# kubagalecki/L3STER

Measured on AMD Instinct MI355X. Metric: DOF/s for MF operator apply (Diffusion3D, hex p=6), higher is better.
Workload: dtype f64

## Files before the change

l3ster_amd/csrc/device/sumfact_fast.hpp:

```cpp
#ifndef L3K_DEVICE_SUMFACT_FAST_HPP
#define L3K_DEVICE_SUMFACT_FAST_HPP

#include "sumfact_apply.hpp"

#include <cstdio>
#include <cstdlib>
#include <type_traits>

namespace l3k::dev
{
template < int NIN, int NOUT, bool ANTI, bool ACC >
__device__ __forceinline__ void sweepEO(const double (&in)[NIN], double (&out)[NOUT], const double* __restrict__ eo)
{
    constexpr int HI = NIN / 2, HO = NOUT / 2, RI = (NIN + 1) / 2, RO = (NOUT + 1) / 2;
    const double* We = eo;
    const double* Wo = eo + RI * RO;
    double        e[RI], o[HI > 0 ? HI : 1];
#pragma unroll
    for (int r = 0; r < HI; ++r)
    {
        e[r] = in[r] + in[NIN - 1 - r];
        o[r] = in[r] - in[NIN - 1 - r];
    }
    if constexpr (NIN % 2)
        e[HI] = in[HI];
#pragma unroll
    for (int q = 0; q < HO; ++q)
    {
        double A = 0.;
#pragma unroll
        for (int r = 0; r < RI; ++r)
            A += e[r] * We[r * RO + q];
        if constexpr (ACC)
        {
            double lo = A;
#pragma unroll
            for (int r = 0; r < HI; ++r)
                lo += o[r] * Wo[r * RO + q];
            out[q] += lo;
            out[NOUT - 1 - q] += ANTI ? lo - 2. * A : 2. * A - lo;
        }
        else
        {
            double lo = A;
#pragma unroll
            for (int r = 0; r < HI; ++r)
                lo += o[r] * Wo[r * RO + q];
            out[q]            = lo;
            out[NOUT - 1 - q] = ANTI ? lo - 2. * A : 2. * A - lo;
        }
    }
    if constexpr (NOUT % 2)
    {
        double m = 0.;
        if constexpr (ANTI)
        {
#pragma unroll
            for (int r = 0; r < HI; ++r)
                m += o[r] * Wo[r * RO + HO];
        }
        else
        {
#pragma unroll
            for (int r = 0; r < RI; ++r)
                m += e[r] * We[r * RO + HO];
        }
        out[HO] = ACC ? out[HO] + m : m;
    }
}

template < int NIN, int NOUT, bool ANTI, bool ACC >
__device__ __forceinline__ void sweepEOSecond(bool live, const double (&in)[NIN], double (&out)[NOUT], const double* __restrict__ eo)
{
    if (live)
        sweepEO< NIN, NOUT, ANTI, ACC >(in, out, eo);
    else if constexpr (!ACC)
    {
#pragma unroll
        for (int q = 0; q < NOUT; ++q)
            out[q] = 0.;
    }
}

template < int N1, int NQ >
struct FastTables
{
    static constexpr int HN = (N1 + 1) / 2, HQ = (NQ + 1) / 2;
    double               eoI[2 * HN * HQ], eoC[2 * HQ * HQ], eoIt[2 * HQ * HN], eoCt[2 * HQ * HQ], qw[NQ], qx[NQ];
};

__device__ __forceinline__ int opaqueZero()
{
    int z;
    asm volatile("s_mov_b32 %0, 0" : "=s"(z) : : "memory");
    return z;
}
__device__ __forceinline__ int opaqueCopy(int x)
{
    int y;
    asm volatile("v_mov_b32 %0, %1" : "=v"(y) : "v"(x));
    return y;
}
__device__ __forceinline__ double opaqueCopy(double x)
{
    double y;
    asm volatile("v_mov_b64 %0, %1" : "=v"(y) : "v"(x));
    return y;
}
template < int N >
__device__ __forceinline__ void loadTable(double (&t)[N], const double* src)
{
#pragma unroll
    for (int i = 0; i < N; ++i)
        t[i] = src[i];
    __builtin_amdgcn_sched_barrier(0);
}
__device__ __forceinline__ void stageFence()
{
    __builtin_amdgcn_fence(__ATOMIC_RELEASE, "wavefront");
    __builtin_amdgcn_wave_barrier();
    __builtin_amdgcn_fence(__ATOMIC_ACQUIRE, "wavefront");
}

#ifdef L3K_ABLATION
#define L3K_STAMP(k)                                                                                                   \
    do                                                                                                                 \
    {                                                                                                                  \
        if (a.stamps != nullptr && blockIdx.x == 0 && stamp_it < 256)                                                  \
        {                                                                                                              \
            const long long t_ = __builtin_readcyclecounter();                                                         \
            if (lane == 0)                                                                                             \
                a.stamps[stamp_it * 16 + (k)] = t_;                                                                    \
        }                                                                                                              \
    } while (0)
#else
#define L3K_STAMP(k)                                                                                                   \
    do                                                                                                                 \
    {                                                                                                                  \
    } while (0)
#endif

#ifndef L3K_FAST_MIN_WAVES
#define L3K_FAST_MIN_WAVES 2
#endif
template < typename K >
constexpr bool kernelUsesFieldDers()
{
    if constexpr (requires { K::field_derivatives; })
        return K::field_derivatives;
    else
        return true;
}

template < int U >
__device__ __forceinline__ uint32_t dirichletBits(const uint8_t* __restrict__ mask, int64_t node)
{
    if constexpr (U == 4)
    {
        const uint32_t w = *reinterpret_cast< const uint32_t* >(mask + node * 4);
        return ((w & 0xffu) ? 1u : 0u) | ((w & 0xff00u) ? 2u : 0u) | ((w & 0xff0000u) ? 4u : 0u) | ((w & 0xff000000u) ? 8u : 0u);
    }
    else if constexpr (U == 2)
    {
        const uint32_t w = *reinterpret_cast< const uint16_t* >(mask + node * 2);
        return ((w & 0xffu) ? 1u : 0u) | ((w & 0xff00u) ? 2u : 0u);
    }
    else
    {
        uint32_t dm = 0;
#pragma unroll
        for (int u = 0; u < U; ++u)
            dm |= uint32_t(mask[node * U + u] != 0) << u;
        return dm;
    }
}

template < typename K, int NQ_, int NFD >
constexpr int kernelWavesPerSimd()
{
    if constexpr (requires { K::waves_per_simd; })
        return K::waves_per_simd;
    else
        return K::params.n_unknowns == 1 && NQ_ * NFD <= 36 ? 3 : L3K_FAST_MIN_WAVES;
}

template < typename K, int P, int NQ >
struct FastCfg
{
    static constexpr int N1 = P + 1, M = cmax(N1, NQ), TEAM = M * M, NN = N1 * N1 * N1;
    static constexpr int U = K::params.n_unknowns, F = K::params.n_fields, NF = U + F;
    static constexpr int NG = (NF + 1) / 2;
    static constexpr int UG = (U + 1) / 2;
    static constexpr int EW = 64 / TEAM > 0 ? 64 / TEAM : 1;
#ifdef L3K_FAST_PS
    static constexpr int PS = M == 7 ? L3K_FAST_PS : M * M, OS = PS * M;
#else
    static constexpr int PS_PAD = M == 8 ? 65 : (M == 6 ? 41 : (M == 4 ? 19 : M * M));
    static constexpr int ldsWith(int ps)
    {
        const int ng = (NF + 1) / 2, dg = kernelUsesFieldDers< K >() ? ng : (U + 1) / 2, os = ps * M;
        const bool alias = dg < ng && ng - dg >= dg;
        return 8 * EW * ((alias ? 2 * ng * os : 2 * ng * os + 2 * dg * os) + 26) + 16 * N1 * N1;
    }
    static constexpr int PS = ldsWith(PS_PAD) <= 64 * 1024 ? PS_PAD : M * M, OS = PS * M;
#endif
    static constexpr int    DG       = kernelUsesFieldDers< K >() ? NG : UG;
    static constexpr int    DF       = kernelUsesFieldDers< K >() ? NF : U;
    static constexpr int    BUF_D    = 2 * NG * OS;
    static constexpr int    BUFB_D   = 2 * DG * OS;
    static constexpr bool   ALIAS_B  = DG < NG && NG - DG >= DG;
    static constexpr int    OFF_B    = ALIAS_B ? 2 * DG * OS : BUF_D;
    static constexpr int    OFF_V    = ALIAS_B ? BUF_D : BUF_D + BUFB_D;
    static constexpr int    TEAM_D   = OFF_V + 24 + 2;
    static constexpr int    SLOT_B   = 16 * N1 * N1;
    static constexpr size_t lds      = sizeof(double) * size_t(EW) * TEAM_D + SLOT_B;
#ifndef L3K_FAST_PS
    static_assert(lds == size_t(ldsWith(PS)));
#endif
    static constexpr int    SG       = (64 / EW) / U * U;
    static constexpr int    NSH      = NN - (N1 - 2) * (N1 - 2) * (N1 - 2);
    static constexpr bool   feasible = TEAM <= 64 && lds <= 64 * 1024 && NF * cmax(N1, NQ) <= 64 && NN * U <= BUFB_D && N1 <= 8 && SG >= U;
    static constexpr int waves_by_lds = int((160 * 1024) / (lds > 0 ? lds : 1));
    static constexpr int min_waves    = waves_by_lds <= 4 ? 1 : (waves_by_lds <= 8 ? cmin(2, kernelWavesPerSimd< K, NQ, NF + DF >()) : kernelWavesPerSimd< K, NQ, NF + DF >());
    static constexpr int wavesPerSimd(bool multi) { return multi ? cmin(2, min_waves) : min_waves; }
    static constexpr int read_block   = NG;
    static constexpr bool multi_column = EW > 1;
};

template < typename K, int P, int NQ, bool SPLIT, bool ENERGY, bool AFFINE = false, bool MULTI = false, bool STRIDED = false, bool RHS = false >
__global__ __launch_bounds__(64, (FastCfg< K, P, NQ >::wavesPerSimd(MULTI))) void sumfactFastKernel(const ElemArgs a, const K kern, int64_t n_batches,
                                                        int xcd_chunk, const FastTables< P + 1, NQ > tab)
{
    using Cfg = FastCfg< K, P, NQ >;
    constexpr int N1 = Cfg::N1, M = Cfg::M, PS = Cfg::PS, OS = Cfg::OS, TEAM = Cfg::TEAM, EW = Cfg::EW;
    constexpr int U = Cfg::U, F = Cfg::F, NF = Cfg::NF, NG = Cfg::NG, UG = Cfg::UG, NN = N1 * N1 * N1;
    constexpr int DG = Cfg::DG, DF = Cfg::DF;
    static_assert(!STRIDED || (!ENERGY && !AFFINE && !MULTI));
    static_assert(!RHS || (!ENERGY && !AFFINE && !MULTI && !STRIDED));
    [[maybe_unused]] const int dpn = a.dofs_per_node;
    auto dirBits = [&](int64_t node) -> uint32_t {
        if constexpr (STRIDED)
        {
            uint32_t dm = 0;
#pragma unroll
            for (int u = 0; u < U; ++u)
                dm |= uint32_t(a.dirichlet[node * dpn + a.field_inds[u]] != 0) << u;
            return dm;
        }
        else
            return dirichletBits< U >(a.dirichlet, node);
    };
#if defined(L3K_FLAGGED_SCATTER)
    constexpr bool ENERGY_AT_END = false;
#elif defined(L3K_ENERGY_AT_END)
    constexpr bool ENERGY_AT_END = L3K_ENERGY_AT_END != 0;
#else
    constexpr bool ENERGY_AT_END = EW == 1;
#endif
    constexpr int HN = (N1 + 1) / 2, HQ = (NQ + 1) / 2;
    constexpr int GB = Cfg::read_block;
    constexpr bool INPLACE = DG < NG;
    auto          at = [](int c, int b, int a_) { return b * PS + a_ * M + c; };

    extern __shared__ double lds[];
    const int                lane = threadIdx.x;
    const int                team = lane / TEAM, l = lane - team * TEAM;
    const bool               worker = team < EW && l < cmax(N1 * N1, cmax(N1 * NQ, NQ * NQ));
    constexpr int            SG     = Cfg::SG;
    double* const            base = lds + size_t(worker ? team : 0) * Cfg::TEAM_D;
    double2* const           bufA = reinterpret_cast< double2* >(base);
    double2* const           bufB = reinterpret_cast< double2* >(base + Cfg::OFF_B);
    double* const            vs   = base + Cfg::OFF_V;

    const double* const eoI  = tab.eoI;
    const double* const eoC  = tab.eoC;
    const double* const eoIt = tab.eoIt;
    const double* const eoCt = tab.eoCt;
    const double* const qw   = tab.qw;
    const double* const qp   = tab.qx;

    const int  i1 = l % N1, j1 = l / N1;
    const bool on_nn = worker && (N1 == NQ ? true : l < N1 * N1);
    const int  iq = l % N1, kq = l / N1;
    const int  qa = l % NQ, qb = l / NQ;

    auto ldg = [&](const double2* buf, int g, int idx) { return buf[g * OS + idx]; };
    auto stg = [&](double2* buf, int g, int idx, double x0, double x1) { buf[g * OS + idx] = make_double2(x0, x1); };

    const int nb     = static_cast< int >(n_batches);
    const int by_xcd = xcd_chunk > 0;
    const int stride = by_xcd ? int(gridDim.x) >> 3 : int(gridDim.x);
    const int first  = by_xcd ? int(blockIdx.x & 7) * xcd_chunk : 0;
    const int last   = by_xcd ? (first + xcd_chunk < nb ? first + xcd_chunk : nb) : nb;
    const bool dyn     = a.work_counters != nullptr;
    const bool sharded = by_xcd || (gridDim.x & 7u) == 0;
    int        victim  = sharded ? int(blockIdx.x & 7u) : 0, switches = 0;
    auto       vBase   = [&](int v) { return by_xcd ? v * xcd_chunk : v; };
    auto       vLimit  = [&](int v) { return by_xcd ? (v * xcd_chunk + xcd_chunk < nb ? v * xcd_chunk + xcd_chunk : nb) : nb; };
    const int  dyn_step = by_xcd || !sharded ? 1 : 8;
    auto       drawTicket = [&]() -> uint32_t {
        uint32_t t = 0;
        if (dyn && lane == 0)
            t = __hip_atomic_fetch_add(a.work_counters + 32 * victim, 1u, __ATOMIC_RELAXED, __HIP_MEMORY_SCOPE_AGENT);
        return t;
    };
    auto ticketBatch = [&](uint32_t t) {
        int b = vBase(victim) + int(__builtin_amdgcn_readfirstlane(t)) * dyn_step;
        while (b >= vLimit(victim))
        {
            if (!by_xcd || ++switches > 7)
                return nb;
            victim = (victim + 1) & 7;
            b      = vBase(victim) + int(__builtin_amdgcn_readfirstlane(drawTicket())) * dyn_step;
        }
        return b;
    };
    const int lim   = dyn ? nb : last;
    int       batch = dyn ? ticketBatch(drawTicket()) : first + (by_xcd ? int(blockIdx.x >> 3) : int(blockIdx.x));
    uint32_t      ids_cur[N1], ids_nxt[N1];
    double        xn[N1][U];
    double        fn[N1][F > 0 ? F : 1];
    uint32_t      dm_nxt[N1];
    const int64_t n_owned_nodes = a.n_owned_dofs / (STRIDED ? a.dofs_per_node : U);
    auto          elemOf = [&](int b) { return a.elem_begin + int64_t(b) * EW + team; };
    auto          valid  = [&](int b) { return (b < lim) & on_nn & ((int64_t(b) * EW + team) < a.elem_count); };
    const bool have_flags = a.elem_flags != nullptr;
    auto       loadIds    = [&](int batch, uint32_t (&ids)[N1], uint32_t& flag) {
        const int lane_o = opaqueCopy(lane), steam = lane_o / SG;
        uint32_t  fg = 0, fs = 0;
        if (have_flags && batch < lim)
        {
            if (steam < EW && (int64_t(batch) * EW + steam) < a.elem_count)
                fs = a.elem_flags[a.elem_begin + int64_t(batch) * EW + steam];
            if constexpr (EW == 1)
                fg = fs;
            else if (worker && (int64_t(batch) * EW + team) < a.elem_count)
                fg = a.elem_flags[elemOf(batch)];
        }
        flag = ((fg & 1u) ? 1u : 0u) | ((fs & 1u) ? 2u : 0u);
        if (valid(batch))
        {
            const uint32_t* en = a.elem_nodes + elemOf(batch) * NN + (lane_o - team * TEAM);
#pragma unroll
            for (int k = 0; k < N1; ++k)
                ids[k] = en[k * N1 * N1];
        }
    };
    [[maybe_unused]] int col = 0;
    auto loadX = [&](bool mine, const uint32_t (&ids)[N1], bool flagged) {
        if (!mine)
            return;
        const double* const ax  = MULTI ? a.x + size_t(col) * a.ldx : a.x;
        const double* const axg = MULTI && SPLIT ? a.xg + size_t(col) * a.ldxg : a.xg;
#pragma unroll
        for (int k = 0; k < N1; ++k)
        {
            const int64_t node = ids[k];
            const double* p    = STRIDED ? (!SPLIT || node < n_owned_nodes ? ax + node * dpn : axg + (node - n_owned_nodes) * dpn)
                                         : (!SPLIT || node < n_owned_nodes ? ax + node * U : axg + (node - n_owned_nodes) * U);
            if constexpr (RHS)
            {
                const uint32_t dm = flagged ? dirBits(node) : 0u;
#pragma unroll
                for (int u = 0; u < U; ++u)
                    xn[k][u] = (dm >> u) & 1u ? a.dirichlet_vals[node * U + u] : 0.;
            }
            else if constexpr (STRIDED)
            {
#pragma unroll
                for (int u = 0; u < U; ++u)
                    xn[k][u] = p[a.field_inds[u]];
            }
            else if constexpr (U % 2 == 0)
            {
#pragma unroll
                for (int hh = 0; hh < U / 2; ++hh)
                {
                    const double2 t = (L3K_DBG(a) & 2) ? make_double2(1e-9 * double(node), 1e-9)
                                                  : *reinterpret_cast< const double2* >(p + 2 * hh);
                    xn[k][2 * hh]     = t.x;
                    xn[k][2 * hh + 1] = t.y;
                }
            }
            else
            {
#pragma unroll
                for (int u = 0; u < U; ++u)
                    xn[k][u] = (L3K_DBG(a) & 2) ? 1e-9 * double(node) : p[u];
            }
            dm_nxt[k] = !RHS && flagged ? dirBits(node) : 0u;
#pragma unroll
            for (int f = 0; f < F; ++f)
                fn[k][f] = a.fields[node + f * a.ldf];
        }
    };

    const double eta_l = qp[qa < NQ ? qa : 0], zeta_l = qp[qb < NQ ? qb : 0];
    const double wyz_l = qw[qa < NQ ? qa : 0] * qw[qb < NQ ? qb : 0];

    uint4* const slotRows = reinterpret_cast< uint4* >(lds + size_t(EW) * Cfg::TEAM_D);
    if (lane < N1 * N1)
        slotRows[lane] = reinterpret_cast< const uint4* >(a.slot_tab)[lane];
    if constexpr (ENERGY)
        if (worker && l == 0)
            vs[24] = 0.;
    stageFence();
    uint32_t flag_cur, flag_nxt = 0;
    loadIds(batch, ids_cur, flag_cur);

    [[maybe_unused]] int stamp_it = 0;
#ifdef L3K_ABLATION
    if (a.stamps != nullptr && blockIdx.x < 4096 && lane == 0)
        a.stamps[256 * 16 + 2 * blockIdx.x] = __builtin_readcyclecounter();
#endif
    while (batch < lim)
    {
        const uint32_t ticket = drawTicket();
        L3K_STAMP(0);
        const bool act = (int64_t(batch) * EW + team) < a.elem_count;
        const bool w_all = worker & act;
        const bool w_nn = N1 == NQ ? w_all : (w_all & (l < N1 * N1)), w_nq = N1 == NQ ? w_all : (w_all & (l < N1 * NQ)),
                   w_qq = N1 == NQ ? w_all : (w_all & (l < NQ * NQ));
        int        batch_next = 0;
        col                   = 0;
        do
        {
        if (w_all)
        {
        loadX(w_nn, ids_cur, RHS ? (a.dirichlet_vals != nullptr && ((flag_cur & 1u) != 0 || !have_flags)) : (flag_cur & 1u) != 0);
        double u0[N1][2 * NG];
        if (w_nn)
        {
#pragma unroll
            for (int k = 0; k < N1; ++k)
            {
#pragma unroll
                for (int u = 0; u < U; ++u)
                    u0[k][u] = xn[k][u];
                if (!RHS && (flag_cur & 1u) != 0)
                {
#pragma unroll
                    for (int u = 0; u < U; ++u)
                        u0[k][u] = (dm_nxt[k] >> u) & 1u ? 0. : u0[k][u];
                }
#pragma unroll
                for (int f = 0; f < F; ++f)
                    u0[k][U + f] = fn[k][f];
                if constexpr (NF % 2)
                    u0[k][NF] = 0.;
            }
        }
        constexpr bool VREG = TEAM >= 24;
        double         vreg = 0.;
        if constexpr (VREG)
        {
            if (l < 24)
                vreg = a.elem_verts[elemOf(batch) * 24 + opaqueCopy(l)];
        }
        else
        {
            for (int t = opaqueCopy(l); t < 24; t += TEAM)
                vs[t] = a.elem_verts[elemOf(batch) * 24 + t];
        }

        if (w_nn)
        {
            double tI[2 * HN * HQ];
            loadTable(tI, eoI + opaqueZero());
#pragma unroll
            for (int g = 0; g < NG; ++g)
            {
                double in0[N1], in1[N1], o0[NQ], o1[NQ];
#pragma unroll
                for (int k = 0; k < N1; ++k)
                {
                    in0[k] = u0[k][2 * g];
                    in1[k] = u0[k][2 * g + 1];
                }
                sweepEO< N1, NQ, false, false >(in0, o0, tI);
                sweepEOSecond< N1, NQ, false, false >(2 * g + 1 < NF, in1, o1, tI);
#pragma unroll
                for (int q = 0; q < NQ; ++q)
                    stg(bufA, g, at(i1, j1, q), o0[q], o1[q]);
            }
        }
        stageFence();
        L3K_STAMP(1);
        if (w_nq)
        {
            double tI[2 * HN * HQ];
            loadTable(tI, eoI + opaqueZero());
#pragma unroll
            for (int gb = 0; gb < NG; gb += GB)
            {
            double in0[GB][N1], in1[GB][N1];
#pragma unroll
            for (int g = gb; g < gb + GB && g < NG; ++g)
#pragma unroll
                for (int j = 0; j < N1; ++j)
                {
                    const double2 t = ldg(bufA, g, at(iq, j, kq));
                    in0[g - gb][j] = t.x;
                    in1[g - gb][j] = t.y;
                }
#pragma unroll
            for (int g = gb; g < gb + GB && g < NG; ++g)
            {
                double o0[NQ], o1[NQ];
                sweepEO< N1, NQ, false, false >(in0[g - gb], o0, tI);
                sweepEOSecond< N1, NQ, false, false >(2 * g + 1 < NF, in1[g - gb], o1, tI);
#pragma unroll
                for (int q = 0; q < NQ; ++q)
                    stg(INPLACE ? bufA : bufB, g, at(iq, q, kq), o0[q], o1[q]);
            }
            }
        }
        stageFence();
        L3K_STAMP(2);
        double v[NQ][2 * NG], dxi[NQ][2 * NG];
        if (w_qq)
        {
            double tI[2 * HN * HQ];
            loadTable(tI, eoI + opaqueZero());
#pragma unroll
            for (int gb = 0; gb < NG; gb += GB)
            {
            double in0[GB][N1], in1[GB][N1];
#pragma unroll
            for (int g = gb; g < gb + GB && g < NG; ++g)
#pragma unroll
                for (int i = 0; i < N1; ++i)
                {
                    const double2 t = ldg(INPLACE ? bufA : bufB, g, at(i, qa, qb));
                    in0[g - gb][i] = t.x;
                    in1[g - gb][i] = t.y;
                }
#pragma unroll
            for (int g = gb; g < gb + GB && g < NG; ++g)
            {
                double o0[NQ], o1[NQ];
                sweepEO< N1, NQ, false, false >(in0[g - gb], o0, tI);
                sweepEOSecond< N1, NQ, false, false >(2 * g + 1 < NF, in1[g - gb], o1, tI);
#pragma unroll
                for (int q = 0; q < NQ; ++q)
                {
                    v[q][2 * g]     = o0[q];
                    v[q][2 * g + 1] = o1[q];
                    if (g < DG)
                        stg(bufA, g, at(q, qa, qb), o0[q], o1[q]);
                }
            }
            }
            double tC[2 * HQ * HQ];
            loadTable(tC, eoC + opaqueZero());
#pragma unroll
            for (int o = 0; o < DF; ++o)
            {
                double in[NQ], der[NQ];
#pragma unroll
                for (int q = 0; q < NQ; ++q)
                    in[q] = v[q][o];
                sweepEO< NQ, NQ, true, false >(in, der, tC);
#pragma unroll
                for (int q = 0; q < NQ; ++q)
                    dxi[q][o] = der[q];
            }
        }
        stageFence();
        L3K_STAMP(3);
        if (w_qq)
        {
            double tC[2 * HQ * HQ];
            loadTable(tC, eoC + opaqueZero());
#pragma unroll
            for (int gb = 0; gb < DG; gb += GB)
            {
            double in0[GB][NQ], in1[GB][NQ];
#pragma unroll
            for (int g = gb; g < gb + GB && g < DG; ++g)
#pragma unroll
                for (int q = 0; q < NQ; ++q)
                {
                    const double2 t = ldg(bufA, g, at(qa, q, qb));
                    in0[g - gb][q] = t.x;
                    in1[g - gb][q] = t.y;
                }
#pragma unroll
            for (int g = gb; g < gb + GB && g < DG; ++g)
            {
                double o0[NQ], o1[NQ];
                sweepEO< NQ, NQ, true, false >(in0[g - gb], o0, tC);
                sweepEOSecond< NQ, NQ, true, false >(2 * g + 1 < DF, in1[g - gb], o1, tC);
#pragma unroll
                for (int q = 0; q < NQ; ++q)
                    stg(bufB, g, at(qa, q, qb), o0[q], o1[q]);
            }
            }
        }
        stageFence();
        L3K_STAMP(4);
        if (w_qq)
        {
            double tC[2 * HQ * HQ];
            loadTable(tC, eoC + opaqueZero());
#pragma unroll
            for (int gb = 0; gb < DG; gb += GB)
            {
            double in0[GB][NQ], in1[GB][NQ];
#pragma unroll
            for (int g = gb; g < gb + GB && g < DG; ++g)
#pragma unroll
                for (int q = 0; q < NQ; ++q)
                {
                    const double2 t = ldg(bufA, g, at(qa, qb, q));
                    in0[g - gb][q] = t.x;
                    in1[g - gb][q] = t.y;
                }
#pragma unroll
            for (int g = gb; g < gb + GB && g < DG; ++g)
            {
                double o0[NQ], o1[NQ];
                sweepEO< NQ, NQ, true, false >(in0[g - gb], o0, tC);
                sweepEOSecond< NQ, NQ, true, false >(2 * g + 1 < DF, in1[g - gb], o1, tC);
#pragma unroll
                for (int q = 0; q < NQ; ++q)
                    stg(bufA, g, at(qa, qb, q), o0[q], o1[q]);
            }
            }
        }
        stageFence();
        L3K_STAMP(5);
        if (w_qq)
        {
            [[maybe_unused]] double en = 0.;
            const double wyz = opaqueCopy(wyz_l) * (ENERGY || RHS ? 1. : a.alpha);
            double       G[6][3];
            if constexpr (VREG && EW == 1)
            {
                double vtx[24];
#pragma unroll
                for (int t = 0; t < 24; ++t)
                {
                    const int lo = __builtin_amdgcn_readlane(__double2loint(vreg), t), hi = __builtin_amdgcn_readlane(__double2hiint(vreg), t);
                    vtx[t]       = __hiloint2double(hi, lo);
                }
                hexPencilGeom(vtx, eta_l, zeta_l, G);
            }
            else
            {
                if constexpr (VREG)
                {
                    if (l < 24)
                        vs[l] = vreg;
                    stageFence();
                }
                hexPencilGeom(vs, eta_l, zeta_l, G);
            }
            {
                [[maybe_unused]] double Jm0[3][3], Ji0[3][3], x0[3], det0 = 0.;
                if constexpr (AFFINE)
                {
                    hexPointOnPencil(G, 0., Jm0, x0);
                    det0 = inverse3(Jm0, Ji0);
                }
#pragma unroll
            for (int q = 0; q < NQ; ++q)
            {
                double vv[NF], dv[3][NF], r0[U], rd[3][U];
#pragma unroll
                for (int g = 0; g < DG; ++g)
                {
                    const double2 te = ldg(bufB, g, at(q, qa, qb)), tz = ldg(bufA, g, at(q, qa, qb));
                    dv[1][2 * g] = te.x;
                    dv[2][2 * g] = tz.x;
                    if (2 * g + 1 < NF)
                    {
                        dv[1][2 * g + 1] = te.y;
                        dv[2][2 * g + 1] = tz.y;
                    }
                }
#pragma unroll
                for (int o = 0; o < NF; ++o)
                {
                    vv[o] = v[q][o];
                    if (o < DF)
                        dv[0][o] = dxi[q][o];
                    else
                        dv[0][o] = dv[1][o] = dv[2][o] = 0.;
                }
                if constexpr (AFFINE)
                {
                    const double xyz[3] = {G[0][0] + qp[q] * G[1][0], G[0][1] + qp[q] * G[1][1], G[0][2] + qp[q] * G[1][2]};
                    qpStageAt< K, 1, RHS, 1, 0, ENERGY && !ENERGY_AT_END >(kern, Ji0, det0, xyz, qw[q] * wyz, a.time, vv, dv, r0, rd, &en, a.ref_z0 != 0);
                }
                else
                    qpStage< K, 1, RHS, 1, 0, ENERGY && !ENERGY_AT_END >(kern, G, qp[q], qw[q] * wyz, a.time, vv, dv, r0, rd, &en, a.ref_z0 != 0);
#pragma unroll
                for (int o = 0; o < U; ++o)
                {
                    v[q][o]   = r0[o];
                    dxi[q][o] = rd[0][o];
                }
#pragma unroll
                for (int g = 0; g < UG; ++g)
                {
                    stg(bufB, g, at(q, qa, qb), rd[1][2 * g], 2 * g + 1 < U ? rd[1][2 * g + 1] : 0.);
                    stg(bufA, g, at(q, qa, qb), rd[2][2 * g], 2 * g + 1 < U ? rd[2][2 * g + 1] : 0.);
                }
            }
            }
            if constexpr (ENERGY && !ENERGY_AT_END)
                atomicAdd(vs + 24, en);
        }
        stageFence();
        L3K_STAMP(6);
        if (w_qq)
        {
            double tCt[2 * HQ * HQ];
            loadTable(tCt, eoCt + opaqueZero());
            double e0[UG][NQ], e1[UG][NQ];
#pragma unroll
            for (int g = 0; g < UG; ++g)
#pragma unroll
                for (int q = 0; q < NQ; ++q)
                {
                    const double2 t = ldg(bufB, g, at(qa, q, qb));
                    e0[g][q] = t.x;
                    e1[g][q] = t.y;
                }
#pragma unroll
            for (int g = 0; g < UG; ++g)
            {
                double o0[NQ], o1[NQ];
                sweepEO< NQ, NQ, true, false >(e0[g], o0, tCt);
                sweepEOSecond< NQ, NQ, true, false >(2 * g + 1 < U, e1[g], o1, tCt);
#pragma unroll
                for (int q = 0; q < NQ; ++q)
                    stg(bufB, g, at(qa, q, qb), o0[q], o1[q]);
            }
            stageFence();
#pragma unroll
            for (int g = 0; g < UG; ++g)
            {
                double z0[NQ], z1[NQ], b0[NQ], b1[NQ];
#pragma unroll
                for (int q = 0; q < NQ; ++q)
                {
                    const double2 t = ldg(bufA, g, at(qa, qb, q));
                    z0[q] = t.x;
                    z1[q] = t.y;
                }
#pragma unroll
                for (int q = 0; q < NQ; ++q)
                {
                    const double2 t = ldg(bufB, g, at(qa, qb, q));
                    b0[q] = t.x;
                    b1[q] = t.y;
                }
                sweepEO< NQ, NQ, true, true >(z0, b0, tCt);
                sweepEOSecond< NQ, NQ, true, true >(2 * g + 1 < U, z1, b1, tCt);
#pragma unroll
                for (int q = 0; q < NQ; ++q)
                    stg(bufB, g, at(qa, qb, q), b0[q], b1[q]);
            }
        }
        stageFence();
        L3K_STAMP(7);
        if (w_qq)
        {
            double tCt[2 * HQ * HQ];
            loadTable(tCt, eoCt + opaqueZero());
#pragma unroll
            for (int g = 0; g < UG; ++g)
            {
                double r10[NQ], r11[NQ], w0[NQ], w1[NQ];
#pragma unroll
                for (int q = 0; q < NQ; ++q)
                {
                    const double2 tb = ldg(bufB, g, at(q, qa, qb));
                    r10[q] = dxi[q][2 * g];
                    r11[q] = dxi[q][2 * g + 1];
                    w0[q]  = v[q][2 * g] + tb.x;
                    w1[q]  = v[q][2 * g + 1] + tb.y;
                }
                sweepEO< NQ, NQ, true, true >(r10, w0, tCt);
                sweepEOSecond< NQ, NQ, true, true >(2 * g + 1 < U, r11, w1, tCt);
#pragma unroll
                for (int q = 0; q < NQ; ++q)
                {
                    v[q][2 * g]     = w0[q];
                    v[q][2 * g + 1] = w1[q];
                }
            }
            double tIt[2 * HQ * HN];
            loadTable(tIt, eoIt + opaqueZero());
#pragma unroll
            for (int g = 0; g < UG; ++g)
            {
                double w0[NQ], w1[NQ], o0[N1], o1[N1];
#pragma unroll
                for (int q = 0; q < NQ; ++q)
                {
                    w0[q] = v[q][2 * g];
                    w1[q] = v[q][2 * g + 1];
                }
                sweepEO< NQ, N1, false, false >(w0, o0, tIt);
                sweepEOSecond< NQ, N1, false, false >(2 * g + 1 < U, w1, o1, tIt);
#pragma unroll
                for (int i = 0; i < N1; ++i)
                    stg(bufB, g, at(i, qa, qb), o0[i], o1[i]);
            }
        }
        stageFence();
        L3K_STAMP(8);
        if (w_nq)
        {
            double tIt[2 * HQ * HN];
            loadTable(tIt, eoIt + opaqueZero());
#pragma unroll
            for (int gb = 0; gb < UG; gb += GB)
            {
            double in0[GB][NQ], in1[GB][NQ];
#pragma unroll
            for (int g = gb; g < gb + GB && g < UG; ++g)
#pragma unroll
                for (int q = 0; q < NQ; ++q)
                {
                    const double2 t = ldg(bufB, g, at(iq, q, kq));
                    in0[g - gb][q] = t.x;
                    in1[g - gb][q] = t.y;
                }
#pragma unroll
            for (int g = gb; g < gb + GB && g < UG; ++g)
            {
                double o0[N1], o1[N1];
                sweepEO< NQ, N1, false, false >(in0[g - gb], o0, tIt);
                sweepEOSecond< NQ, N1, false, false >(2 * g + 1 < U, in1[g - gb], o1, tIt);
#pragma unroll
                for (int j = 0; j < N1; ++j)
                    stg(bufA, g, at(iq, j, kq), o0[j], o1[j]);
            }
            }
        }
        stageFence();
        L3K_STAMP(9);
        if (w_nn)
        {
            double tIt[2 * HQ * HN];
            loadTable(tIt, eoIt + opaqueZero());
            double*       sb  = reinterpret_cast< double* >(bufB);
            [[maybe_unused]] double              en_e  = 0.;
            [[maybe_unused]] const double* const ax_e  = a.x;
            [[maybe_unused]] const double* const axg_e = a.xg;
            const uint4   srow = slotRows[l];
            const uint32_t sw[4] = {srow.x, srow.y, srow.z, srow.w};
#pragma unroll
            for (int gb = 0; gb < UG; gb += GB)
            {
            double in0[GB][NQ], in1[GB][NQ];
#pragma unroll
            for (int g = gb; g < gb + GB && g < UG; ++g)
#pragma unroll
                for (int q = 0; q < NQ; ++q)
                {
                    const double2 t = ldg(bufA, g, at(i1, j1, q));
                    in0[g - gb][q] = t.x;
                    in1[g - gb][q] = t.y;
                }
#pragma unroll
            for (int g = gb; g < gb + GB && g < UG; ++g)
            {
                double o0[N1], o1[N1];
                sweepEO< NQ, N1, false, false >(in0[g - gb], o0, tIt);
                sweepEOSecond< NQ, N1, false, false >(2 * g + 1 < U, in1[g - gb], o1, tIt);
#ifndef L3K_FLAGGED_SCATTER
                if (!RHS && (flag_cur & 1u) != 0)
#else
                if (false)
#endif
                {
#pragma unroll
                    for (int k = 0; k < N1; ++k)
                    {
                        const int64_t  node = static_cast< uint32_t >(opaqueCopy(static_cast< int >(ids_cur[k])));
                        const uint32_t dmk  = dirBits(node) >> (2 * g);
                        o0[k]               = (dmk & 1u) ? 0. : o0[k];
                        o1[k]               = (dmk & 2u) ? 0. : o1[k];
                    }
                }
#pragma unroll
                for (int k = 0; k < N1; ++k)
                {
                    const uint32_t slot = (k & 1) ? sw[k >> 1] >> 16 : sw[k >> 1] & 0xffffu;
                    double*        dstl = sb + slot * U + 2 * g;
                    if constexpr (U % 2 == 0)
                        *reinterpret_cast< double2* >(dstl) = ENERGY ? make_double2(a.alpha * o0[k], a.alpha * o1[k]) : make_double2(o0[k], o1[k]);
                    else
                    {
                        dstl[0] = ENERGY ? a.alpha * o0[k] : o0[k];
                        if (2 * g + 1 < U)
                            dstl[1] = ENERGY ? a.alpha * o1[k] : o1[k];
                    }
                }
                if constexpr (ENERGY && ENERGY_AT_END)
                {
#pragma unroll
                    for (int k = 0; k < N1; ++k)
                    {
                        const int64_t node = static_cast< uint32_t >(opaqueCopy(static_cast< int >(ids_cur[k])));
                        const double* px   = (!SPLIT || node < n_owned_nodes ? ax_e + node * U : axg_e + (node - n_owned_nodes) * U) + 2 * g;
                        if constexpr (U % 2 == 0)
                        {
                            const double2 xv = *reinterpret_cast< const double2* >(px);
                            en_e += xv.x * o0[k] + xv.y * o1[k];
                        }
                        else
                        {
                            en_e += px[0] * o0[k];
                            if (2 * g + 1 < U)
                                en_e += px[1] * o1[k];
                        }
                    }
                }
            }
            }
            if constexpr (ENERGY && ENERGY_AT_END)
                atomicAdd(vs + 24, en_e);
        }
        stageFence();
        L3K_STAMP(10);
        if (w_nn)
        {
            uint32_t* const idsL = reinterpret_cast< uint32_t* >(bufA);
            const uint4     srow = slotRows[l];
            const uint32_t  sw[4] = {srow.x, srow.y, srow.z, srow.w};
#pragma unroll
            for (int k = 0; k < N1; ++k)
                idsL[(k & 1) ? sw[k >> 1] >> 16 : sw[k >> 1] & 0xffffu] = ids_cur[k];
        }
        }
        stageFence();
        L3K_STAMP(11);
        if (!MULTI || col == (a.n_cols > 1 ? a.n_cols : 1) - 1)
        {
            batch_next = dyn ? ticketBatch(ticket) : batch + stride;
            loadIds(batch_next, ids_nxt, flag_nxt);
        }
        double* const ay  = MULTI ? a.y + size_t(col) * a.ldy : a.y;
        double* const ayg = MULTI && SPLIT ? a.yg + size_t(col) * a.ldyg : a.yg;
        const int lane_s = opaqueCopy(lane);
        const int steam_s = lane_s / SG, sl = lane_s - steam_s * SG;
        if (steam_s < EW && (int64_t(batch) * EW + steam_s) < a.elem_count)
        {
            const double* const   sb      = lds + size_t(steam_s) * Cfg::TEAM_D + Cfg::OFF_B;
            const uint32_t* const idsS    = reinterpret_cast< const uint32_t* >(lds + size_t(steam_s) * Cfg::TEAM_D);
#ifndef L3K_FLAGGED_SCATTER
            constexpr bool        flagged = false;
#else
            const bool            flagged = (flag_cur & 2u) != 0;
#endif
            static_assert(SG % U == 0);
            constexpr int         XW = U % 2 == 0 ? 2 : 1, UX = U / XW;
            using xval_t = std::conditional_t< XW == 2, double2, double >;
            const int             sl_node = sl / U, sl_o = sl % U, sl_node2 = sl / UX, sl_o2 = XW * (sl % UX);
            [[maybe_unused]] const int sl_f = STRIDED ? a.field_inds[sl_o] : sl_o;
            const uint32_t* const ids1 = idsS + sl_node;
            const double* const   sb1  = sb + sl;
            const uint32_t* const ids2 = idsS + sl_node2;
            const xval_t* const   sb2  = reinterpret_cast< const xval_t* >(sb) + sl;
            auto shellRound = [&]< int NSH_, bool FLAGGED >(int r) {
                if ((r + 1) * SG > NSH_ * U && r * SG + sl >= NSH_ * U)
                    return;
                if ((L3K_DBG(a) & 128) && (r & 1))
                    return;
                const int64_t node = ids1[r * (SG / U)];
                const int64_t dof  = STRIDED ? node * dpn + sl_f : node * U + sl_o;
                const double  val  = sb1[r * SG];
                double*       dst  = !SPLIT || node < n_owned_nodes ? ay + dof : ayg + (dof - a.n_owned_dofs);
                if constexpr (FLAGGED)
                    if (a.dirichlet[dof] != 0)
                        return;
                if (L3K_DBG(a) & (1 | 32 | 64))
                {
                    if ((L3K_DBG(a) & 32) || val == 1.2345e300)
                        *dst = val;
                }
                else if (L3K_DBG(a) & 16)
                    *dst += val;
                else
                    unsafeAtomicAdd(dst, val);
            };
            auto exclStore = [&](double* dst, xval_t out) {
                if constexpr (XW == 2)
                {
                    if (a.beta != 0.)
                    {
                        const double2 old = *reinterpret_cast< const double2* >(dst);
                        out.x += a.beta * old.x;
                        out.y += a.beta * old.y;
                    }
                    *reinterpret_cast< double2* >(dst) = out;
                }
                else
                    *dst = a.beta != 0. ? out + a.beta * *dst : out;
            };
            auto exclRound = [&]< int NSH_, bool FLAGGED >(int r) {
                if (NSH_ * UX + r * SG + sl >= NN * UX)
                    return;
                const int64_t node = ids2[NSH_ + r * (SG / UX)];
                const int64_t dof  = node * U + sl_o2;
                const xval_t  val  = sb2[NSH_ * UX + r * SG];
                double*       dst  = ay + dof;
                xval_t        out  = val;
                if constexpr (FLAGGED)
                {
                    if constexpr (XW == 2)
                    {
                        out.x = a.dirichlet[dof] != 0 ? 0. : val.x;
                        out.y = a.dirichlet[dof + 1] != 0 ? 0. : val.y;
                    }
                    else
                        out = a.dirichlet[dof] != 0 ? 0. : val;
                }
                if (L3K_DBG(a) & 1)
                {
                    double first;
                    if constexpr (XW == 2)
                        first = val.x;
                    else
                        first = val;
                    if (first == 1.2345e300)
                        *dst = first;
                    return;
                }
                exclStore(dst, out);
            };
            constexpr int RS = (Cfg::NSH * U + SG - 1) / SG, RX = ((NN - Cfg::NSH) * UX + SG - 1) / SG;
            if (!STRIDED && !RHS && a.fuse_beta && !flagged)
            {
#ifdef L3K_ABLATION
#pragma unroll
                for (int r = 0; r < RS; ++r)
                    shellRound.template operator()< Cfg::NSH, false >(r);
#pragma unroll
                for (int r = 0; r < RX; ++r)
                    exclRound.template operator()< Cfg::NSH, false >(r);
#else
                constexpr int  NSHU = Cfg::NSH * U, NXH = (NN - Cfg::NSH) * UX;
                uint32_t       nid[RS], nid2[RX > 0 ? RX : 1];
                double         val[RS];
                xval_t         val2[RX > 0 ? RX : 1];
                constexpr bool part1 = RS * SG > NSHU, part2 = RX * SG > NXH;
                const bool     in1 = !part1 || (RS - 1) * SG + sl < NSHU, in2 = !part2 || (RX - 1) * SG + sl < NXH;
#pragma unroll
                for (int r = 0; r < RS; ++r)
                {
                    nid[r] = ids1[r * (SG / U)];
                    val[r] = sb1[r * SG];
                }
#pragma unroll
                for (int r = 0; r < RX; ++r)
                    if (r + 1 < RX || in2)
                    {
                        nid2[r] = ids2[Cfg::NSH + r * (SG / UX)];
                        val2[r] = sb2[Cfg::NSH * UX + r * SG];
                    }
#pragma unroll
                for (int r = 0; r < RS; ++r)
                    if (r + 1 < RS || in1)
                    {
                        const int64_t node = nid[r];
                        const int64_t dof  = node * U + sl_o;
                        double*       dst  = !SPLIT || node < n_owned_nodes ? ay + dof : ayg + (dof - a.n_owned_dofs);
                        unsafeAtomicAdd(dst, val[r]);
                    }
#pragma unroll
                for (int r = 0; r < RX; ++r)
                    if (r + 1 < RX || in2)
                    {
                        exclStore(ay + int64_t(nid2[r]) * U + sl_o2, val2[r]);
                    }
#endif
            }
            else if (!STRIDED && !RHS && a.fuse_beta)
            {
#pragma unroll 1
                for (int r = 0; r < RS; ++r)
                    shellRound.template operator()< Cfg::NSH, true >(r);
#pragma unroll 1
                for (int r = 0; r < RX; ++r)
                    exclRound.template operator()< Cfg::NSH, true >(r);
            }
            else if (!flagged)
            {
#pragma unroll 1
                for (int r = 0; r < (NN * U + SG - 1) / SG; ++r)
                    shellRound.template operator()< NN, false >(r);
            }
            else
            {
#pragma unroll 1
                for (int r = 0; r < (NN * U + SG - 1) / SG; ++r)
                    shellRound.template operator()< NN, true >(r);
            }
        }
        stageFence();
        L3K_STAMP(12);
        } while (MULTI && ++col < a.n_cols);
#pragma unroll
        for (int k = 0; k < N1; ++k)
            ids_cur[k] = ids_nxt[k];
        flag_cur = flag_nxt;
        batch    = batch_next;
        ++stamp_it;
// ... 172 lines not shown
```

l3ster_amd/csrc/user_kernels.hpp:

```cpp
#ifndef L3K_USER_KERNELS_HPP
#define L3K_USER_KERNELS_HPP

#include "l3k/kernel_interface.hpp"

#include <cmath>

namespace l3k::kernels
{
struct Diffusion3D
{
    static constexpr KernelParams params{.dimension = 3, .n_equations = 7, .n_unknowns = 4};
    double                        k = 1., s = 1.;

    template < typename In, typename Out >
    L3K_HD void operator()(const In&, Out& out) const
    {
        auto& [operators, rhs] = out;
        auto& [A0, Ax, Ay, Az] = operators;
        Ax(0, 1) = -k;
        Ay(0, 2) = -k;
        Az(0, 3) = -k;
        rhs[0]   = s;
        A0(1, 1) = -1.;
        Ax(1, 0) = 1.;
        A0(2, 2) = -1.;
        Ay(2, 0) = 1.;
        A0(3, 3) = -1.;
        Az(3, 0) = 1.;
        Ay(4, 3) = 1.;
        Az(4, 2) = -1.;
        Ax(5, 3) = -1.;
        Az(5, 1) = 1.;
        Ax(6, 2) = 1.;
        Ay(6, 1) = -1.;
    }
};

struct Diffusion3DVar
{
    static constexpr KernelParams params{.dimension = 3, .n_equations = 7, .n_unknowns = 4, .n_fields = 1};

    template < typename In, typename Out >
    L3K_HD void operator()(const In& in, Out& out) const
    {
        const auto& [field_vals, field_ders, _] = in;
        const auto lambda                       = field_vals[0];
        const auto& [dx, dy, dz]                = field_ders;
        const auto dl_dx                        = dx[0];
        const auto dl_dy                        = dy[0];
        const auto dl_dz                        = dz[0];

        auto& [operators, rhs] = out;
        auto& [A0, Ax, Ay, Az] = operators;
        A0(0, 1) = -dl_dx;
        A0(0, 2) = -dl_dy;
        A0(0, 3) = -dl_dz;
        Ax(0, 1) = -lambda;
        Ay(0, 2) = -lambda;
        Az(0, 3) = -lambda;
        A0(1, 1) = -1.;
        Ax(1, 0) = 1.;
        A0(2, 2) = -1.;
        Ay(2, 0) = 1.;
        A0(3, 3) = -1.;
        Az(3, 0) = 1.;
        Ay(4, 3) = 1.;
        Az(4, 2) = -1.;
        Ax(5, 3) = -1.;
        Az(5, 1) = 1.;
        Ax(6, 2) = 1.;
        Ay(6, 1) = -1.;
    }
};

struct AdvDiff3D
{
    static constexpr KernelParams params{.dimension = 3, .n_equations = 7, .n_unknowns = 4, .n_fields = 3};
    static constexpr bool         field_derivatives = false;
    double                        k = 1., sigma = 1., s = 1.;

    template < typename In, typename Out >
    L3K_HD void operator()(const In& in, Out& out) const
    {
        const auto& [u, u_ders, point] = in;
        auto& [operators, rhs]         = out;
        auto& [A0, Ax, Ay, Az]         = operators;
        A0(0, 0) = sigma;
        Ax(0, 0) = u[0];
        Ay(0, 0) = u[1];
        Az(0, 0) = u[2];
        Ax(0, 1) = -k;
        Ay(0, 2) = -k;
        Az(0, 3) = -k;
        rhs[0]   = s;
        A0(1, 1) = -1.;
        Ax(1, 0) = 1.;
        A0(2, 2) = -1.;
        Ay(2, 0) = 1.;
        A0(3, 3) = -1.;
        Az(3, 0) = 1.;
        Ay(4, 3) = 1.;
        Az(4, 2) = -1.;
        Ax(5, 3) = -1.;
        Az(5, 1) = 1.;
        Ax(6, 2) = 1.;
        Ay(6, 1) = -1.;
    }
};

struct Diffusion3DPoint
{
    static constexpr KernelParams params{.dimension = 3, .n_equations = 7, .n_unknowns = 4};
    double                        k = 1., s = 1.;

    template < typename In, typename Out >
    L3K_HD void operator()(const In& in, Out& out) const
    {
        const auto& [field_vals, field_ders, point] = in;
        const double x = point.space.x(), y = point.space.y(), z = point.space.z(), t = point.time;
        const double kv = k * (1. + 0.3 * sin(x + 2. * y + 3. * z + t));
        const double c  = -(1. + 0.2 * cos(z - t));

        auto& [operators, rhs] = out;
        auto& [A0, Ax, Ay, Az] = operators;
        Ax(0, 1) = -kv;
        Ay(0, 2) = -kv;
        Az(0, 3) = -kv;
        rhs[0]   = s * (1. + x * y - 0.5 * z * t);
        A0(1, 1) = c;
        Ax(1, 0) = 1.;
        A0(2, 2) = c;
        Ay(2, 0) = 1.;
        A0(3, 3) = c;
        Az(3, 0) = 1.;
        Ay(4, 3) = 1.;
        Az(4, 2) = -1.;
        Ax(5, 3) = -1.;
        Az(5, 1) = 1.;
        Ax(6, 2) = 1.;
        Ay(6, 1) = -1.;
    }
};

struct Advection3D
{
    static constexpr KernelParams params{.dimension = 3, .n_equations = 1, .n_unknowns = 1, .n_fields = 3};
    static constexpr bool         field_derivatives = false;
    double                        dt = .02;

    template < typename In, typename Out >
    L3K_HD void operator()(const In& in, Out& out) const
    {
        const auto& [field_vals, field_ders, point] = in;
        const double y_scaled = point.space.y() * 2. - 1., z_scaled = point.space.z() * 2. - 1.;
        const double vx = (1. - y_scaled * y_scaled) * (1. - .5 * z_scaled * z_scaled);
        const double vy = .25 * point.space.x();
        const double vz = -.125;

        constexpr double bdf_leading_coef = 11. / 6.;
        constexpr double bdf_coefs[3]     = {3., -1.5, 1. / 3.};

        auto& [operators, rhs] = out;
        auto& [A0, A1, A2, A3] = operators;
        A0(0, 0) = bdf_leading_coef;
        A1(0, 0) = vx * dt;
        A2(0, 0) = vy * dt;
        A3(0, 0) = vz * dt;
        rhs[0]   = field_vals[0] * bdf_coefs[0] + field_vals[1] * bdf_coefs[1] + field_vals[2] * bdf_coefs[2];
    }
};

struct DivCurl3D
{
    static constexpr KernelParams params{.dimension = 3, .n_equations = 4, .n_unknowns = 3};
    double                        f = 1.;

    template < typename In, typename Out >
    L3K_HD void operator()(const In& in, Out& out) const
    {
        const double a         = 1. + .5 * in.point.space.x() * in.point.space.z();
        auto& [operators, rhs] = out;
        auto& [A0, Ax, Ay, Az] = operators;
        Ax(0, 0) = a;
        Ay(0, 1) = a;
        Az(0, 2) = a;
        rhs[0]   = f;
        Ay(1, 2) = 1.;
        Az(1, 1) = -1.;
        Az(2, 0) = 1.;
        Ax(2, 2) = -1.;
        Ax(3, 1) = 1.;
        Ay(3, 0) = -1.;
        A0(1, 0) = .1 * in.point.space.y();
        rhs[1]   = .5;
    }
};

struct Mass3D
{
    static constexpr KernelParams params{.dimension = 3, .n_equations = 2, .n_unknowns = 2};

    template < typename In, typename Out >
    L3K_HD void operator()(const In&, Out& out) const
    {
        auto& [operators, rhs] = out;
        auto& [A0, Ax, Ay, Az] = operators;
        A0(0, 0) = 1.;
        A0(1, 1) = 1.;
        rhs[0]   = 1.;
        rhs[1]   = 2.;
    }
};

struct Adiabatic3D
{
    static constexpr KernelParams params{.dimension = 3, .n_equations = 1, .n_unknowns = 4};

    template < typename In, typename Out >
    L3K_HD void operator()(const In& in, Out& out) const
    {
        const auto& [vals, ders, point, normal] = in;
        auto& [operators, rhs]                  = out;
        auto& [A0, A1, A2, A3]                  = operators;
        A0(0, 1) = normal[0];
        A0(0, 2) = normal[1];
        A0(0, 3) = normal[2];
    }
};
struct Robin3D
{
    static constexpr KernelParams params{.dimension = 3, .n_equations = 1, .n_unknowns = 4};
    double                        h = 1., t_inf = 0.;

    template < typename In, typename Out >
    L3K_HD void operator()(const In& in, Out& out) const
    {
        const auto& [vals, ders, point, normal] = in;
        auto& [operators, rhs]                  = out;
        auto& [A0, A1, A2, A3]                  = operators;
        A0(0, 0) = h;
        A0(0, 1) = normal[0];
        A0(0, 2) = normal[1];
        A0(0, 3) = normal[2];
        rhs[0]   = h * t_inf;
    }
};

struct RobinPoint3D
{
    static constexpr KernelParams params{.dimension = 3, .n_equations = 1, .n_unknowns = 4};
    double                        h0 = 1., t0 = 0.;

    template < typename In, typename Out >
    L3K_HD void operator()(const In& in, Out& out) const
    {
        const auto& [vals, ders, point, normal] = in;
        const double h         = h0 * (1. + .5 * sin(point.space.x() - point.space.y() + point.time));
        auto& [operators, rhs] = out;
        auto& [A0, A1, A2, A3] = operators;
        A0(0, 0) = h;
        A0(0, 1) = normal[0];
        A0(0, 2) = normal[1];
        A0(0, 3) = normal[2];
        rhs[0]   = h * t0 * (1. + point.space.z());
    }
// ... 302 lines not shown
```

Measured before the change: 89.17 billion.

## Prefetch next element's node ids, DOF gather and vertices during current element's backward sweeps

Adds a gather-ahead path for single-element-per-wave p=6/NQ=7 configurations. The next batch's ticket and node ids are drawn mid-way through the current element's backward sum-factorization sweeps, and its DOF values, fields and vertex coordinates are gathered into registers during the remaining sweeps. The aim is to hide global-memory gather latency behind compute. Dirichlet bit lookup moves to the consuming iteration, and a waitcnt is placed before the scatter. The cost is extra live registers, which may lower occupancy. Diffusion3DPoint opts out.

```diff
diff --git a/l3ster_amd/csrc/device/sumfact_fast.hpp b/l3ster_amd/csrc/device/sumfact_fast.hpp
--- a/l3ster_amd/csrc/device/sumfact_fast.hpp
+++ b/l3ster_amd/csrc/device/sumfact_fast.hpp
@@ -107,6 +107,8 @@
     asm volatile("v_mov_b64 %0, %1" : "=v"(y) : "v"(x));
     return y;
 }
+__device__ __forceinline__ void anyValue(uint32_t& x) { asm("" : "=v"(x)); }
+__device__ __forceinline__ void anyValue(double& x) { asm("" : "=v"(x)); }
 template < int N >
 __device__ __forceinline__ void loadTable(double (&t)[N], const double* src)
 {
@@ -182,6 +184,15 @@
         return K::waves_per_simd;
     else
         return K::params.n_unknowns == 1 && NQ_ * NFD <= 36 ? 3 : L3K_FAST_MIN_WAVES;
+}
+
+template < typename K >
+constexpr bool kernelGathersAhead()
+{
+    if constexpr (requires { K::gather_ahead; })
+        return K::gather_ahead;
+    else
+        return true;
 }
 
 template < typename K, int P, int NQ >
@@ -225,6 +236,7 @@
     static constexpr int wavesPerSimd(bool multi) { return multi ? cmin(2, min_waves) : min_waves; }
     static constexpr int read_block   = NG;
     static constexpr bool multi_column = EW > 1;
+    static constexpr bool gather_ahead = EW == 1 && N1 == 7 && NQ == 7 && SG == 64 && kernelGathersAhead< K >();
 };
 
 template < typename K, int P, int NQ, bool SPLIT, bool ENERGY, bool AFFINE = false, bool MULTI = false, bool STRIDED = false, bool RHS = false >
@@ -237,6 +249,11 @@
     constexpr int DG = Cfg::DG, DF = Cfg::DF;
     static_assert(!STRIDED || (!ENERGY && !AFFINE && !MULTI));
     static_assert(!RHS || (!ENERGY && !AFFINE && !MULTI && !STRIDED));
+#if defined(L3K_FLAGGED_SCATTER) || defined(L3K_ABLATION)
+    constexpr bool GA = false;
+#else
+    constexpr bool GA = Cfg::gather_ahead && !MULTI && !STRIDED && !RHS;
+#endif
     [[maybe_unused]] const int dpn = a.dofs_per_node;
     auto dirBits = [&](int64_t node) -> uint32_t {
         if constexpr (STRIDED)
@@ -301,7 +318,7 @@
     auto       drawTicket = [&]() -> uint32_t {
         uint32_t t = 0;
         if (dyn && lane == 0)
-            t = __hip_atomic_fetch_add(a.work_counters + 32 * victim, 1u, __ATOMIC_RELAXED, __HIP_MEMORY_SCOPE_AGENT);
+            t = __hip_atomic_fetch_add(a.work_counters + 32 * victim + (GA ? opaqueCopy(0) : 0), 1u, __ATOMIC_RELAXED, __HIP_MEMORY_SCOPE_AGENT);
         return t;
     };
     auto ticketBatch = [&](uint32_t t) {
@@ -321,6 +338,7 @@
     double        xn[N1][U];
     double        fn[N1][F > 0 ? F : 1];
     uint32_t      dm_nxt[N1];
+    [[maybe_unused]] double vreg_nxt = 0.;
     const int64_t n_owned_nodes = a.n_owned_dofs / (STRIDED ? a.dofs_per_node : U);
     auto          elemOf = [&](int b) { return a.elem_begin + int64_t(b) * EW + team; };
     auto          valid  = [&](int b) { return (b < lim) & on_nn & ((int64_t(b) * EW + team) < a.elem_count); };
@@ -338,7 +356,23 @@
                 fg = a.elem_flags[elemOf(batch)];
         }
         flag = ((fg & 1u) ? 1u : 0u) | ((fs & 1u) ? 2u : 0u);
-        if (valid(batch))
+        if constexpr (GA)
+        {
+            if (batch < lim)
+            {
+                const uint32_t* en = a.elem_nodes + (a.elem_begin + int64_t(batch)) * NN + (lane_o < N1 * N1 ? lane_o : N1 * N1 - 1);
+#pragma unroll
+                for (int k = 0; k < N1; ++k)
+                    ids[k] = en[k * N1 * N1];
+            }
+            else
+            {
+#pragma unroll
+                for (int k = 0; k < N1; ++k)
+                    anyValue(ids[k]);
+            }
+        }
+        else if (valid(batch))
         {
             const uint32_t* en = a.elem_nodes + elemOf(batch) * NN + (lane_o - team * TEAM);
 #pragma unroll
@@ -388,10 +422,33 @@
                 for (int u = 0; u < U; ++u)
                     xn[k][u] = (L3K_DBG(a) & 2) ? 1e-9 * double(node) : p[u];
             }
-            dm_nxt[k] = !RHS && flagged ? dirBits(node) : 0u;
+            if constexpr (!GA)
+                dm_nxt[k] = !RHS && flagged ? dirBits(node) : 0u;
 #pragma unroll
             for (int f = 0; f < F; ++f)
                 fn[k][f] = a.fields[node + f * a.ldf];
+        }
+    };
+    [[maybe_unused]] auto gatherAhead = [&](int b, const uint32_t (&ids)[N1]) {
+        if (b < lim)
+        {
+            loadX(true, ids, false);
+            const int lane_o = opaqueCopy(lane);
+            vreg_nxt         = a.elem_verts[(a.elem_begin + int64_t(b)) * 24 + (lane_o < 24 ? lane_o : 23)];
+        }
+        else
+        {
+#pragma unroll
+            for (int k = 0; k < N1; ++k)
+            {
+#pragma unroll
+                for (int u = 0; u < U; ++u)
+                    anyValue(xn[k][u]);
+#pragma unroll
+                for (int f = 0; f < F; ++f)
+                    anyValue(fn[k][f]);
+            }
+            anyValue(vreg_nxt);
         }
     };
 
@@ -407,6 +464,8 @@
     stageFence();
     uint32_t flag_cur, flag_nxt = 0;
     loadIds(batch, ids_cur, flag_cur);
+    if constexpr (GA)
+        gatherAhead(batch, ids_cur);
 
     [[maybe_unused]] int stamp_it = 0;
 #ifdef L3K_ABLATION
@@ -425,9 +484,11 @@
         col                   = 0;
         do
         {
+        double v[NQ][2 * NG], dxi[NQ][2 * NG];
         if (w_all)
         {
-        loadX(w_nn, ids_cur, RHS ? (a.dirichlet_vals != nullptr && ((flag_cur & 1u) != 0 || !have_flags)) : (flag_cur & 1u) != 0);
+        if constexpr (!GA)
+            loadX(w_nn, ids_cur, RHS ? (a.dirichlet_vals != nullptr && ((flag_cur & 1u) != 0 || !have_flags)) : (flag_cur & 1u) != 0);
         double u0[N1][2 * NG];
         if (w_nn)
         {
@@ -439,6 +500,8 @@
                     u0[k][u] = xn[k][u];
                 if (!RHS && (flag_cur & 1u) != 0)
                 {
+                    if constexpr (GA)
+                        dm_nxt[k] = dirBits(ids_cur[k]);
 #pragma unroll
                     for (int u = 0; u < U; ++u)
                         u0[k][u] = (dm_nxt[k] >> u) & 1u ? 0. : u0[k][u];
@@ -452,7 +515,9 @@
         }
         constexpr bool VREG = TEAM >= 24;
         double         vreg = 0.;
-        if constexpr (VREG)
+        if constexpr (VREG && GA)
+            vreg = vreg_nxt;
+        else if constexpr (VREG)
         {
             if (l < 24)
                 vreg = a.elem_verts[elemOf(batch) * 24 + opaqueCopy(l)];
@@ -517,7 +582,6 @@
         }
         stageFence();
         L3K_STAMP(2);
-        double v[NQ][2 * NG], dxi[NQ][2 * NG];
         if (w_qq)
         {
             double tI[2 * HN * HQ];
@@ -813,6 +877,14 @@
         }
         stageFence();
         L3K_STAMP(8);
+        }
+        if constexpr (GA)
+        {
+            batch_next = dyn ? ticketBatch(ticket) : batch + stride;
+            loadIds(batch_next, ids_nxt, flag_nxt);
+        }
+        if (w_all)
+        {
         if (w_nq)
         {
             double tIt[2 * HQ * HN];
@@ -844,6 +916,11 @@
         }
         stageFence();
         L3K_STAMP(9);
+        }
+        if constexpr (GA)
+            gatherAhead(batch_next, ids_nxt);
+        if (w_all)
+        {
         if (w_nn)
         {
             double tIt[2 * HQ * HN];
@@ -941,7 +1018,9 @@
         }
         stageFence();
         L3K_STAMP(11);
-        if (!MULTI || col == (a.n_cols > 1 ? a.n_cols : 1) - 1)
+        if constexpr (GA)
+            __builtin_amdgcn_s_waitcnt(0x0f70);
+        if (!GA && (!MULTI || col == (a.n_cols > 1 ? a.n_cols : 1) - 1))
         {
             batch_next = dyn ? ticketBatch(ticket) : batch + stride;
             loadIds(batch_next, ids_nxt, flag_nxt);
@@ -949,8 +1028,8 @@
         double* const ay  = MULTI ? a.y + size_t(col) * a.ldy : a.y;
         double* const ayg = MULTI && SPLIT ? a.yg + size_t(col) * a.ldyg : a.yg;
         const int lane_s = opaqueCopy(lane);
-        const int steam_s = lane_s / SG, sl = lane_s - steam_s * SG;
-        if (steam_s < EW && (int64_t(batch) * EW + steam_s) < a.elem_count)
+        const int steam_s = GA ? 0 : lane_s / SG, sl = lane_s - steam_s * SG;
+        if (GA || (steam_s < EW && (int64_t(batch) * EW + steam_s) < a.elem_count))
         {
             const double* const   sb      = lds + size_t(steam_s) * Cfg::TEAM_D + Cfg::OFF_B;
             const uint32_t* const idsS    = reinterpret_cast< const uint32_t* >(lds + size_t(steam_s) * Cfg::TEAM_D);
@@ -959,7 +1038,7 @@
 #else
             const bool            flagged = (flag_cur & 2u) != 0;
 #endif
-            static_assert(SG % U == 0);
+            static_assert(SG % U == 0 && (!GA || SG == 64));
             constexpr int         XW = U % 2 == 0 ? 2 : 1, UX = U / XW;
             using xval_t = std::conditional_t< XW == 2, double2, double >;
             const int             sl_node = sl / U, sl_o = sl % U, sl_node2 = sl / UX, sl_o2 = XW * (sl % UX);
diff --git a/l3ster_amd/csrc/user_kernels.hpp b/l3ster_amd/csrc/user_kernels.hpp
--- a/l3ster_amd/csrc/user_kernels.hpp
+++ b/l3ster_amd/csrc/user_kernels.hpp
@@ -111,6 +111,7 @@
 struct Diffusion3DPoint
 {
     static constexpr KernelParams params{.dimension = 3, .n_equations = 7, .n_unknowns = 4};
+    static constexpr bool         gather_ahead = false;
     double                        k = 1., s = 1.;
 
     template < typename In, typename Out >
```

Measured after the change: 92.07 billion (median of 6 runs). 1.03x the previous value.
